# uthree/tinyvc

Measured on AMD Instinct MI355X. Metric: audio-samples/sec (16 kHz) end-to-end VC, higher is better.
Workload: dtype f32 (fp32 in / out / accumulate; channel contractions as two-term fp16 splits on v_mfma_f32_32x32x16_f16: 22-bit significands, three part-products per fp32 product)

## Files before the change

### tinyvc_amd/csrc/conv48s.hip

```cpp
#include "small_kernels.h"
#include "split_fp16.h"
#include "tvc_common.h"

namespace tvc {

namespace {

constexpr int kC48 = 48, kBN48 = 128, kXP48 = kBN48 + 2 * 27, kNT48 = 512;
typedef float f32x4s_t __attribute__((ext_vector_type(4)));
typedef unsigned u32x2_t __attribute__((ext_vector_type(2)));

__device__ __forceinline__ void split4_48(const float (&v)[4], u32x2_t& p1, u32x2_t& p2) {
#pragma unroll
    for (int j = 0; j < 2; ++j) {
        unsigned q1, q2;
        split2(v[2 * j], v[2 * j + 1], q1, q2);
        p1[j] = q1;
        p2[j] = q2;
    }
}

__device__ __forceinline__ void ld8_g8(float (&dst)[8], const float* base, unsigned byte_off) {
    const uint4* b4 = reinterpret_cast<const uint4*>(base);
    const f32x4s_t q0 = __builtin_bit_cast(f32x4s_t, ldg_so4(b4, byte_off)), q1 = __builtin_bit_cast(f32x4s_t, ldg_so4(b4, byte_off + 16u));
    dst[0] = q0.x; dst[1] = q0.y; dst[2] = q0.z; dst[3] = q0.w;
    dst[4] = q1.x; dst[5] = q1.y; dst[6] = q1.z; dst[7] = q1.w;
}
__device__ __forceinline__ void ld4_g8(float (&dst)[4], const float* base, unsigned byte_off) {
    const f32x4s_t q0 = __builtin_bit_cast(f32x4s_t, ldg_so4(reinterpret_cast<const uint4*>(base), byte_off));
    dst[0] = q0.x; dst[1] = q0.y; dst[2] = q0.z; dst[3] = q0.w;
}

struct Conv48Args {
    const float* x;
    const float* cond;
    const float* res;
    float* out;
    const u32x4* A6;
    const u32x4* F6;
    const u32x4* W5;
    const float* b5;
    float* out5;
    const float* bias;
    const float* bsc;
    const float* bsh;
    const float* wsc;
    const float* fsc;
    const float* w5sc;
    const float* amax_x;
    const float* amax_c;
    float* amax_y;
    int len, dil, tiles_per_utt, ntiles;
    RagDev rag;
};

template <bool FILM, bool C5 = false, bool RAG = false>
__global__ __launch_bounds__(kNT48) __attribute__((amdgpu_waves_per_eu(FILM ? 2 : 4))) void conv48s_kernel(Conv48Args a) {
    constexpr int C = kC48, BN = kBN48, XP = kXP48, NT = kNT48;
    extern __shared__ __attribute__((aligned(16))) uint4 smem_q[];
    u32x4* Xs = reinterpret_cast<u32x4*>(smem_q);
// ... 8 lines not shown
    const int XW = BN + 2 * dil;
    int bh = 0;
    auto utt = [&](int tile) __attribute__((always_inline)) { return rag_tile<RAG>(a.rag, tile, a.tiles_per_utt, rs, bh).b; };

    for (int i = tid; i < 36 * 64; i += NT) Wt[i] = a.A6[i];
    if (FILM)
        for (int i = tid; i < 24 * 64; i += NT) Ft[i] = a.F6[i];
    if (C5) {
        for (int i = tid; i < 6 * 64; i += NT) W5t[i] = a.W5[i];
        if (tid < 32) Bi[192 + tid] = a.b5[tid];
        if (tid == 0) Bi[224] = 0.f;
    }
    if (tid < 64) {
        const int tc = tid < C ? tid : C - 1;
        Bi[tid] = a.bias[tc];
        if (FILM) {
            Bi[64 + tid] = a.bsc[tc];
            Bi[128 + tid] = a.bsh[tc];
        }
    }
    const float cw = a.wsc[mt], cwsc = FILM ? a.fsc[mt] : 1.f, cwsh = FILM ? a.fsc[2 + mt] : 1.f, cw5 = C5 ? a.w5sc[0] : 1.f;

    constexpr int XPER = 3;
    float xr0[XPER][8];
    int ig[XPER], ic[XPER];
#pragma unroll
    for (int i = 0; i < XPER; ++i) {
        const int idx = tid + i * NT;
        const int g = idx / XW;
        ic[i] = idx - g * XW;
        ig[i] = g;
    }
    auto fetch = [&](int tile) __attribute__((always_inline)) {
        const RagTile rt = rag_tile<RAG>(a.rag, tile, a.tiles_per_utt, rs, bh);
        const int len = rt.len;
        const int px0 = rt.tin * BN - dil;
        const float* xb = RAG ? a.x + 8L * rt.off : a.x + (long)rt.b * C * rs;
#pragma unroll
        for (int i = 0; i < XPER; ++i) {
            const int g = ig[i] > 5 ? 5 : ig[i];
            int p = px0 + ic[i];
            p = p < 0 ? 0 : (p > len - 1 ? len - 1 : p);
            ld8_g8(xr0[i], xb, 32u * (unsigned)(g * rs + p));
        }
    };
    auto deposit = [&](float xs) __attribute__((always_inline)) {
#pragma unroll
        for (int i = 0; i < XPER; ++i) {
            if (ig[i] > 5) continue;
            float v[8];
#pragma unroll
            for (int j = 0; j < 8; ++j) {
                const float t = xr0[i][j];
                v[j] = fmaxf(t, 0.1f * t) * xs;
            }
            uint4 p1, p2;
            split8(v, p1, p2);
            Xs[(0 + ig[i]) * XP + ic[i]] = __builtin_bit_cast(u32x4, p1);
            Xs[(6 + ig[i]) * XP + ic[i]] = __builtin_bit_cast(u32x4, p2);
        }
    };

    int tile, tend;
    tile_range(a.ntiles, tile, tend);
    if (tile >= tend) return;
    bh = utt(tile);
    fetch(tile);
    deposit(bfp_load_u(a.amax_x, bh).s);
    slab_barrier();
    float mx_run = 0.f;
    int mx_b = bh;
    int sc_b = -1;
    Bfp sx{1.f, 1.f}, sc{1.f, 1.f};

    for (; tile < tend; ++tile) {
        const RagTile rt = rag_tile<RAG>(a.rag, tile, a.tiles_per_utt, rs, bh);
        const int b = rt.b, len = rt.len;
        bh = b;
        if (a.amax_y && b != mx_b) {
            amax_flush_wg(a.amax_y + mx_b, mx_run, Bi + 228);
            mx_run = 0.f;
            mx_b = b;
        }
        if (b != sc_b) {
            sc_b = b;
            sx = bfp_load_u(a.amax_x, b);
            sc = FILM ? bfp_load_u(a.amax_c, b) : Bfp{1.f, 1.f};
        }
        const int t0 = rt.tin * BN;
        const int next = tile + 1;
        const int n = nt * 32 + l31;
        const int t = t0 + n;
        const int tc = t < len ? t : len - 1;

        float cr[FILM ? 3 : 1][8];
        if (FILM) {
            const float* cb = RAG ? a.cond + 8L * rt.off : a.cond + (long)b * C * rs;
            const unsigned oc = 32u * (unsigned)(lh * rs + tc);
#pragma unroll
            for (int s = 0; s < 3; ++s) ld8_g8(cr[s], cb + (long)s * 16 * rs, oc);
        }
        float rv[FILM ? 4 : 1][4];
        if constexpr (FILM) {
            const float* rb = RAG ? a.res + 8L * rt.off : a.res + (long)b * C * rs;
            const unsigned og = 32u * (unsigned)(4 * mt * rs + tc) + 16u * (unsigned)lh;
#pragma unroll
            for (int g = 0; g < 4; ++g) {
                if (32 * mt + 8 * g < C) {
                    ld4_g8(rv[g], rb + (long)g * 8 * rs, og);
// ... 52 lines not shown
#pragma unroll
                for (int p = 0; p < 2; ++p) {
                    fa[0][p] = __builtin_bit_cast(f16x8, Ft[((s * 4 + mt) * 2 + p) * 64 + lane]);
                    fa[1][p] = __builtin_bit_cast(f16x8, Ft[((s * 4 + 2 + mt) * 2 + p) * 64 + lane]);
                }
                lsc = TVC_MFMA16(fa[0][1], cf[0], lsc);
                lsh = TVC_MFMA16(fa[1][1], cf[0], lsh);
                asc = TVC_MFMA16(fa[0][0], cf[0], asc);
                ash = TVC_MFMA16(fa[1][0], cf[0], ash);
                lsc = TVC_MFMA16(fa[0][0], cf[1], lsc);
                lsh = TVC_MFMA16(fa[1][0], cf[1], lsh);
            }
            const float c1 = cwsc * sc.inv, c2 = cwsh * sc.inv;
#pragma unroll
            for (int r = 0; r < 16; ++r) {
                asc[r] = comb(asc[r], lsc[r], c1, c1 * kLoInv);
                ash[r] = comb(ash[r], lsh[r], c2, c2 * kLoInv);
            }
        }

        float xv[C5 ? 4 : 1][4];
        float mx = 0.f;
        {
            float* ob = C5 ? nullptr : (RAG ? a.out + 8L * rt.off : a.out + (long)b * C * rs);
            const unsigned og = 32u * (unsigned)(4 * mt * rs + tc) + 16u * (unsigned)lh;
#pragma unroll
            for (int g = 0; g < 4; ++g) {
                if (32 * mt + 8 * g >= C) continue;
                float v4[4];
                const f32x4s_t bv = *reinterpret_cast<const f32x4s_t*>(Bi + 32 * mt + 8 * g + 4 * lh);
                f32x4s_t bs, bh;
                if (FILM) {
                    bs = *reinterpret_cast<const f32x4s_t*>(Bi + 64 + 32 * mt + 8 * g + 4 * lh);
                    bh = *reinterpret_cast<const f32x4s_t*>(Bi + 128 + 32 * mt + 8 * g + 4 * lh);
                }
#pragma unroll
                for (int q = 0; q < 4; ++q) {
                    float v = acc[4 * g + q] + bv[q];
                    if (FILM) {
                        v = __fadd_rn(__fmul_rn(v, asc[4 * g + q] + bs[q]), ash[4 * g + q] + bh[q]);
                        v = __fadd_rn(v, rv[g][q]);
                    }
                    v4[q] = v;
                    if (C5) {
                        xv[g][q] = v;
                        mx = fmaxf(mx, fabsf(v));
                    }
                }
                if (!C5 && t < len) {
                    stg_so4(ob + (long)g * 8 * rs, og, v4);
                    mx = fmaxf(mx, fmaxf(fmaxf(fabsf(v4[0]), fabsf(v4[1])), fmaxf(fabsf(v4[2]), fabsf(v4[3]))));
                }
            }
        }
        if (!C5) mx_run = fmaxf(mx_run, mx);
        if (C5) {
            {
#pragma unroll
                for (int o = 32; o > 0; o >>= 1) mx = fmaxf(mx, __shfl_xor(mx, o));
                if (lane == 0) atomicMax(reinterpret_cast<unsigned*>(Bi + 224), __builtin_bit_cast(unsigned, mx));
            }
            slab_barrier();
            const Bfp s5 = bfp_from_amax(Bi[224]);
#pragma unroll
            for (int g = 0; g < 4; ++g) {
                if (32 * mt + 8 * g >= C) continue;
                u32x2_t p1, p2;
#pragma unroll
                for (int q = 0; q < 4; ++q) xv[g][q] *= s5.s;
                split4_48(xv[g], p1, p2);
                const auto sx_ = __builtin_amdgcn_permlane32_swap(p1[0], p2[0], false, false);
                const auto sy_ = __builtin_amdgcn_permlane32_swap(p1[1], p2[1], false, false);
                const u32x4 row = {sx_[0], sy_[0], sx_[1], sy_[1]};
                *reinterpret_cast<u32x4*>(Xs + (6 * lh + 4 * mt + g) * XP + n) = row;
// ... 19 lines not shown
                float m5 = 0.f;
                if (t < len) {
                    float* o5 = RAG ? a.out5 + 8L * rt.off : a.out5 + (long)b * 24 * rs;
                    const unsigned o5o = 32u * (unsigned)t + 16u * (unsigned)lh;
                    const float c = cw5 * s5.inv, cl = c * kLoInv;
#pragma unroll
                    for (int g = 0; g < 3; ++g) {
                        const f32x4s_t b5v = *reinterpret_cast<const f32x4s_t*>(Bi + 192 + 8 * g + 4 * lh);
                        float v4[4];
#pragma unroll
                        for (int q = 0; q < 4; ++q) {
                            v4[q] = comb(a5[4 * g + q], l5[4 * g + q], c, cl) + b5v[q];
                            m5 = fmaxf(m5, fabsf(v4[q]));
                        }
                        stg_so4(o5 + (long)g * 8 * rs, o5o, v4);
                    }
                }
                mx_run = fmaxf(mx_run, m5);
            }
        }
        slab_barrier();
        if (next < tend) {
            const int bn = utt(next);
            deposit(bn == b ? sx.s : bfp_load_u(a.amax_x, bn).s);
        }
        slab_barrier();
    }
    if (a.amax_y) amax_flush_wg(a.amax_y + mx_b, mx_run, Bi + 228);
}

template <bool FILM, bool C5 = false>
int launch48(tvc_ctx* ctx, hipStream_t s, Conv48Args a, int B) {
    constexpr size_t lds = (size_t)(12 * kXP48 + 36 * 64 + (FILM ? 24 * 64 : 0) + (C5 ? 6 * 64 : 0)) * 16 + 240 * 4;
    TVC_CHECK((lds_optin<conv48s_kernel<FILM, C5>, conv48s_kernel<FILM, C5, true>>(ctx, (int)lds, "conv48s")));
    a.tiles_per_utt = (a.len + kBN48 - 1) / kBN48;
    a.ntiles = a.tiles_per_utt * B;
    TVC_CHECK(rag_tiles(ctx, s, B, a.len, kBN48, &a.rag, &a.ntiles, "conv48s"));
    const int wpc = FILM ? 1 : 2;
    const int grid = a.ntiles < wpc * ctx->ncu ? a.ntiles : wpc * ctx->ncu;
    if (ctx->rag) hipLaunchKernelGGL((conv48s_kernel<FILM, C5, true>), dim3(grid), dim3(kNT48), lds, s, a);
    else hipLaunchKernelGGL((conv48s_kernel<FILM, C5>), dim3(grid), dim3(kNT48), lds, s, a);
    return launch_check(ctx, "conv48s");
}

struct Conv48PArgs {
    const float* x;
    const float* cond;
    float* out;
    const u32x4* Aa;
    const u32x4* Ab;
    const u32x4* F6;
    const float *bias_a, *bias_b, *bsc, *bsh;
    const float *wsc_a, *wsc_b, *fsc;
    const float* amax_x;
    const float* amax_c;
    float* amax_y;
    RagDev rag;
    int len, da, db, lin, tiles_per_utt, ntiles;
    float lscale;
};
constexpr int kXPP = 136;

template <bool FILM, bool RAG = false>
__global__ __launch_bounds__(kNT48) __attribute__((amdgpu_waves_per_eu(2))) void conv48p_kernel(Conv48PArgs a) {
    constexpr int C = kC48, NT = kNT48, XP = kXPP, HP = 128;
    extern __shared__ __attribute__((aligned(16))) uint4 smem_p[];
    u32x4* Xs = reinterpret_cast<u32x4*>(smem_p);
    u32x4* Hs = Xs + 12 * XP;
    u32x4* Wa = Hs + 12 * HP;
    u32x4* Wb = Wa + 36 * 64;
    u32x4* Ft = Wb + 36 * 64;
    float* Bi = reinterpret_cast<float*>(Ft + (FILM ? 24 * 64 : 0));
    const int tid = threadIdx.x, lane = tid & 63, wave = tid >> 6;
    const int l31 = lane & 31, lh = lane >> 5;
    const int mt = wave >> 2, nt = wave & 3;
    const int rs = a.len, da = a.da, db = a.db;
    const int BNO = 128 - 2 * db;
    const int XW = 128 + 2 * da;
    const int rsl = FILM ? a.lin : rs;
    const int xf = FILM ? rs / a.lin : 1;
    int bh = 0;
    auto utt = [&](int tile) __attribute__((always_inline)) { return rag_tile<RAG>(a.rag, tile, a.tiles_per_utt, rs, bh).b; };

    for (int i = tid; i < 36 * 64; i += NT) {
        Wa[i] = a.Aa[i];
        Wb[i] = a.Ab[i];
    }
    if (FILM)
        for (int i = tid; i < 24 * 64; i += NT) Ft[i] = a.F6[i];
    if (tid < 64) {
        const int tc = tid < C ? tid : C - 1;
        Bi[tid] = a.bias_a[tc];
        Bi[64 + tid] = a.bias_b[tc];
        if (FILM) {
            Bi[128 + tid] = a.bsc[tc];
            Bi[192 + tid] = a.bsh[tc];
        }
    }
    if (tid == 0) Bi[256] = 0.f;
    const int mtu = __builtin_amdgcn_readfirstlane(mt);
    const float cwa = a.wsc_a[mtu], cwb = a.wsc_b[mtu], cwsc = FILM ? a.fsc[mtu] : 1.f, cwsh = FILM ? a.fsc[2 + mtu] : 1.f;

    constexpr int XPER = 2;
    float xr0[XPER][8], xr1[FILM ? XPER : 1][8], lam[FILM ? XPER : 1];
    int ig[XPER], ic[XPER];
#pragma unroll
    for (int i = 0; i < XPER; ++i) {
        const int idx = tid + i * NT;
        const int g = idx / XW;
        ic[i] = idx - g * XW;
        ig[i] = g;
    }
    auto fetch = [&](int tile) __attribute__((always_inline)) {
        const RagTile rt = rag_tile<RAG>(a.rag, tile, a.tiles_per_utt, rs, bh);
        const int len = rt.len, lin = FILM ? len / xf : len;
        const int px0 = rt.tin * BNO - db - da;
        const float* xb = RAG ? a.x + (FILM ? 8L * (rt.off / xf) : rt.off) : a.x + (long)rt.b * C * rsl;
#pragma unroll
        for (int i = 0; i < XPER; ++i) {
            const int g = ig[i] > 5 ? 5 : ig[i];
            int p = px0 + ic[i];
            p = p < 0 ? 0 : (p > len - 1 ? len - 1 : p);
// ... 20 lines not shown
            float v[8];
#pragma unroll
            for (int j = 0; j < 8; ++j) {
                float t = FILM ? fmaf(1.f - lam[i], xr0[i][j], __fmul_rn(lam[i], xr1[i][j])) : xr0[i][j];
                v[j] = fmaxf(t, 0.1f * t) * xs;
            }
            uint4 p1, p2;
            split8(v, p1, p2);
            Xs[(0 + g) * XP + c] = __builtin_bit_cast(u32x4, p1);
            Xs[(6 + g) * XP + c] = __builtin_bit_cast(u32x4, p2);
        }
    };

    int tile, tend;
    tile_range(a.ntiles, tile, tend);
    if (tile >= tend) return;
    bh = utt(tile);
    fetch(tile);
    deposit(bfp_load_u(a.amax_x, bh).s);
    slab_barrier();
    float mx_run = 0.f;
    int mx_b = bh;
    int sc_b = -1;
    Bfp sx{1.f, 1.f}, sc{1.f, 1.f};

    for (; tile < tend; ++tile) {
        const RagTile rt = rag_tile<RAG>(a.rag, tile, a.tiles_per_utt, rs, bh);
        const int b = rt.b, len = rt.len;
        bh = b;
        if (a.amax_y && b != mx_b) {
            amax_flush_wg(a.amax_y + mx_b, mx_run, Bi + 260);
            mx_run = 0.f;
            mx_b = b;
        }
        if (b != sc_b) {
            sc_b = b;
            sx = bfp_load_u(a.amax_x, b);
            sc = FILM ? bfp_load_u(a.amax_c, b) : Bfp{1.f, 1.f};
        }
        const int t0 = rt.tin * BNO;
        const int next = tile + 1;
        const int n = nt * 32 + l31;
        const int t = t0 + n;
        const bool live = n < BNO && t < len;
        const int tc = t < len ? t : len - 1;
        const unsigned oo = 4u * (unsigned)((32 * mt + 4 * lh) * rs + tc);

        float cr[FILM ? 3 : 1][8];
        if (FILM) {
            const float* cb = RAG ? a.cond + 8L * rt.off : a.cond + (long)b * C * rs;
            const unsigned oc = 32u * (unsigned)(lh * rs + tc);
#pragma unroll
            for (int s = 0; s < 3; ++s) ld8_g8(cr[s], cb + (long)s * 16 * rs, oc);
        }
        float rv[FILM ? 4 : 1][4];
        if constexpr (FILM) {
            const float* rb = RAG ? a.x + 8L * (rt.off / xf) : a.x + (long)b * C * a.lin;
            const Lerp lc = lerp_coord(tc, a.lscale, RAG ? len / xf : a.lin);
            const unsigned o0 = 32u * (unsigned)(4 * mt * a.lin + lc.i0) + 16u * (unsigned)lh, o1 = 32u * (unsigned)(4 * mt * a.lin + lc.i1) + 16u * (unsigned)lh;
#pragma unroll
// ... 15 lines not shown
            f16x8 af[2][2], bf[2][2];
            auto frags = [&](int s, int fb) __attribute__((always_inline)) {
                const int sl = s / 3, tap = s - sl * 3;
                const int row = (2 * sl + lh) * XP + n + tap * da;
#pragma unroll
                for (int p = 0; p < 2; ++p) {
                    bf[fb][p] = __builtin_bit_cast(f16x8, Xs[p * 6 * XP + row]);
                    af[fb][p] = __builtin_bit_cast(f16x8, Wa[((s * 2 + mt) * 2 + p) * 64 + lane]);
                }
            };
            frags(0, 0);
#pragma unroll
            for (int s = 0; s < 9; ++s) {
                const int fb = s & 1;
                if (s + 1 < 9) frags(s + 1, fb ^ 1);
                __builtin_amdgcn_sched_barrier(0);
                alo = TVC_MFMA16(af[fb][1], bf[fb][0], alo);
                acc = TVC_MFMA16(af[fb][0], bf[fb][0], acc);
                alo = TVC_MFMA16(af[fb][0], bf[fb][1], alo);
                __builtin_amdgcn_sched_barrier(0);
            }
        }
        fetch(next < tend ? next : tile);
        float hv[4][4];
        float hmx = 0.f;
        {
            const float c = cwa * sx.inv, cl = c * kLoInv;
#pragma unroll
            for (int g = 0; g < 4; ++g) {
                const f32x4s_t bv = *reinterpret_cast<const f32x4s_t*>(Bi + 32 * mt + 8 * g + 4 * lh);
#pragma unroll
                for (int q = 0; q < 4; ++q) {
                    const float v = comb(acc[4 * g + q], alo[4 * g + q], c, cl) + bv[q];
                    hv[g][q] = fmaxf(v, 0.1f * v);
                    if (32 * mt + 8 * g < C) hmx = fmaxf(hmx, fabsf(hv[g][q]));
                }
            }
            hmx = wave_max(hmx);
            if (lane == 0) atomicMax(reinterpret_cast<unsigned*>(Bi + 256), __builtin_bit_cast(unsigned, hmx));
        }
        slab_barrier();
        const Bfp sh_ = bfp_from_amax(Bi[256]);
#pragma unroll
        for (int g = 0; g < 4; ++g) {
            if (32 * mt + 8 * g >= C) continue;
            u32x2_t p1, p2;
#pragma unroll
            for (int q = 0; q < 4; ++q) hv[g][q] *= sh_.s;
            split4_48(hv[g], p1, p2);
            const auto sx_ = __builtin_amdgcn_permlane32_swap(p1[0], p2[0], false, false);
            const auto sy_ = __builtin_amdgcn_permlane32_swap(p1[1], p2[1], false, false);
            const u32x4 row = {sx_[0], sy_[0], sx_[1], sy_[1]};
            *reinterpret_cast<u32x4*>(Hs + (6 * lh + 4 * mt + g) * HP + n) = row;
        }
        slab_barrier();
        if (tid == 0) Bi[256] = 0.f;

#pragma unroll
        for (int r = 0; r < 16; ++r) acc[r] = alo[r] = 0.f;
        {
            const int lo = db - t0 > 0 ? db - t0 : 0;
            const int hi = len - 1 - t0 + db < HP - 1 ? len - 1 - t0 + db : HP - 1;
            int col[3];
#pragma unroll
            for (int tap = 0; tap < 3; ++tap) {
                int c = n + tap * db;
                c = c > HP - 1 ? HP - 1 : c;
                col[tap] = c < lo ? lo : (c > hi ? hi : c);
            }
            f16x8 af[2][2], bf[2][2];
            auto frags = [&](int s, int fb) __attribute__((always_inline)) {
                const int sl = s / 3, tap = s - sl * 3;
                const int row = (2 * sl + lh) * HP + col[tap];
#pragma unroll
                for (int p = 0; p < 2; ++p) {
                    bf[fb][p] = __builtin_bit_cast(f16x8, Hs[p * 6 * HP + row]);
                    af[fb][p] = __builtin_bit_cast(f16x8, Wb[((s * 2 + mt) * 2 + p) * 64 + lane]);
                }
            };
// ... 64 lines not shown
                for (int q = 0; q < 4; ++q) {
                    float v = acc[4 * g + q] + bv[q];
                    if (FILM) {
                        v = __fadd_rn(__fmul_rn(v, asc[4 * g + q] + bs[q]), ash[4 * g + q] + bh[q]);
                        v = __fadd_rn(v, rv[g][q]);
                    }
                    v4[q] = v;
                    if (!FILM && live) stg_so(ob + (long)(8 * g + q) * rs, oo, v);
                }
                if (live) {
                    if (FILM) stg_so4(ob + (long)g * 8 * rs, og, v4);
                    mx = fmaxf(mx, fmaxf(fmaxf(fabsf(v4[0]), fabsf(v4[1])), fmaxf(fabsf(v4[2]), fabsf(v4[3]))));
                }
            }
            mx_run = fmaxf(mx_run, mx);
        }
        slab_barrier();
        if (next < tend) {
            const int bn = utt(next);
            deposit(bn == b ? sx.s : bfp_load_u(a.amax_x, bn).s);
        }
        slab_barrier();
    }
    if (a.amax_y) amax_flush_wg(a.amax_y + mx_b, mx_run, Bi + 260);
}

template <bool FILM>
int launch48p(tvc_ctx* ctx, hipStream_t s, Conv48PArgs a, int B) {
    constexpr size_t lds = (size_t)(12 * kXPP + 12 * 128 + 72 * 64 + (FILM ? 24 * 64 : 0)) * 16 + 272 * 4;
    static_assert(lds <= 160 * 1024, "LDS");
    TVC_CHECK((lds_optin<conv48p_kernel<FILM>, conv48p_kernel<FILM, true>>(ctx, (int)lds, "conv48p")));
    const int bno = 128 - 2 * a.db;
    a.tiles_per_utt = (a.len + bno - 1) / bno;
    a.ntiles = a.tiles_per_utt * B;
    TVC_CHECK(rag_tiles(ctx, s, B, a.len, bno, &a.rag, &a.ntiles, "conv48p"));
    const int grid = a.ntiles < ctx->ncu ? a.ntiles : ctx->ncu;
    if (ctx->rag) hipLaunchKernelGGL((conv48p_kernel<FILM, true>), dim3(grid), dim3(kNT48), lds, s, a);
    else hipLaunchKernelGGL((conv48p_kernel<FILM>), dim3(grid), dim3(kNT48), lds, s, a);
    return launch_check(ctx, "conv48p");
}

}

int run_conv48s(tvc_ctx* ctx, hipStream_t s, const PackedW& w, const float* x, const PackedW* film, const float* bsc, const float* bsh,
                const float* cond, const float* res, float* out, int B, int len, int dil, const float* amax_x, const float* amax_c, float* amax_y,
                const PackedW* c5, float* out5) {
    if (w.cin != kC48 || w.M != kC48 || w.taps != 3 || w.MT6 != 2 || !w.A6) return fail(ctx, TVC_ERR_ARG, "conv48s: 48 -> 48 channel k3 convs only");
    if (dil < 1 || dil > 27) return fail(ctx, TVC_ERR_ARG, "conv48s: dilation must be 1..27");
    if ((long)len * kC48 * 4 >= (1L << 32)) return fail(ctx, TVC_ERR_ARG, "conv48s: utterance too long for 32-bit byte offsets");
    if (film && (film->MT6 != 4 || !film->A6 || !cond || !bsc || !bsh)) return fail(ctx, TVC_ERR_ARG, "conv48s: FiLM needs the stacked image, both biases and cond");
    Conv48Args a{};
    a.x = x; a.cond = cond; a.res = res; a.out = out;
    a.A6 = reinterpret_cast<const u32x4*>(w.A6);
    a.F6 = film ? reinterpret_cast<const u32x4*>(film->A6) : nullptr;
    a.bias = w.bias; a.bsc = bsc; a.bsh = bsh;
    a.wsc = w.wscale;
    a.fsc = film ? film->wscale : nullptr;
    a.amax_x = amax_x; a.amax_c = amax_c; a.amax_y = amax_y;
    a.len = len; a.dil = dil;
    if (film) {
        if (!res) return fail(ctx, TVC_ERR_ARG, "conv48s: the FiLM variants carry a residual");
        if (c5) {
            if (!out5 || c5->M != 24 || c5->cin != kC48 || c5->taps != 1 || c5->MT6 != 1 || !c5->A6)
                return fail(ctx, TVC_ERR_ARG, "conv48s: the fused c5 is the 48 -> 24 1x1 after the second FiLM");
            a.W5 = reinterpret_cast<const u32x4*>(c5->A6);
            a.b5 = c5->bias;
            a.w5sc = c5->wscale;
            a.out5 = out5;
            return launch48<true, true>(ctx, s, a, B);
        }
        return launch48<true>(ctx, s, a, B);
    }
    if (res) return fail(ctx, TVC_ERR_ARG, "conv48s: plain convs carry no residual");
    return launch48<false>(ctx, s, a, B);
}

int run_conv48_pair(tvc_ctx* ctx, hipStream_t s, const PackedW& wa, const PackedW& wb, const float* x, int lin, float lscale, const PackedW* film,
                    const float* bsc, const float* bsh, const float* cond, float* out, int B, int len, int da, int db, const float* amax_x,
                    const float* amax_c, float* amax_y) {
    for (const PackedW* w : {&wa, &wb})
        if (w->cin != kC48 || w->M != kC48 || w->taps != 3 || w->MT6 != 2 || !w->A6) return fail(ctx, TVC_ERR_ARG, "conv48 pair: 48 -> 48 channel k3 convs only");
    if (da < 1 || da > 4 || db < 1 || db > 8) return fail(ctx, TVC_ERR_ARG, "conv48 pair: dilations (1..4, 1..8)");
    if ((long)len * kC48 * 4 >= (1L << 32)) return fail(ctx, TVC_ERR_ARG, "conv48 pair: utterance too long for 32-bit byte offsets");
    if (film && (film->MT6 != 4 || !film->A6 || !cond || !bsc || !bsh))
        return fail(ctx, TVC_ERR_ARG, "conv48 pair: the FiLM variant needs the stacked image, both biases and cond");
    Conv48PArgs a{};
    a.x = x; a.cond = cond; a.out = out;
    a.Aa = reinterpret_cast<const u32x4*>(wa.A6);
    a.Ab = reinterpret_cast<const u32x4*>(wb.A6);
    a.F6 = film ? reinterpret_cast<const u32x4*>(film->A6) : nullptr;
    a.bias_a = wa.bias; a.bias_b = wb.bias; a.bsc = bsc; a.bsh = bsh;
    a.wsc_a = wa.wscale; a.wsc_b = wb.wscale; a.fsc = film ? film->wscale : nullptr;
    a.amax_x = amax_x; a.amax_c = amax_c; a.amax_y = amax_y;
    a.len = len; a.da = da; a.db = db; a.lin = lin; a.lscale = lscale;
    if (film) return lin > 0 ? launch48p<true>(ctx, s, a, B) : fail(ctx, TVC_ERR_ARG, "conv48 pair: the FiLM pair starts from the low-rate tensor");
    if (lin > 0) return fail(ctx, TVC_ERR_ARG, "conv48 pair: the plain pair has no interpolated input");
    return launch48p<false>(ctx, s, a, B);
}

}
```

### tinyvc_amd/csrc/decoder.hip

```cpp
#include "conv3s.h"
#include "conv_s2.h"
#include "film_s2.h"
#include "gemm_s2.h"
#include "small_kernels.h"
#include "tvc_common.h"

namespace tvc {


__device__ __forceinline__ float div24k(float x) {
    const float r = 1.0f / 24000.0f;
    const float q0 = __fmul_rn(x, r);
    return fmaf(fmaf(-q0, 24000.0f, x), r, q0);
}

__device__ __forceinline__ double wave_incl_scan(double v, int lane) {
#pragma unroll
    for (int o = 1; o < 64; o <<= 1) {
        double u = __shfl_up(v, o);
        if (lane >= o) v += u;
    }
    return v;
}

// ... 329 lines not shown
            }
            TVC_CHECK(fk->end());
        }
        TVC_CHECK(run_down0_split(ctx, s, ctx->flt_down0s, source, energy, skip[0], taps ? taps->skips[0] : nullptr, xi_pre[1], B, (int)L, smax, slot(S_SKIP0)));
    }
    for (int i = 1; i <= 4; ++i) {
        const DownW& d = ctx->downs[i - 1];
        const int len = (int)len_dn[i];
        size_t mk = ws.mark();
        float* xi = xi_pre[i];
        float* h1 = d.cin == 24 ? nullptr : ws.get<float>((size_t)B * d.cin * len);
        float* h2 = d.cin == 24 ? nullptr : ws.get<float>((size_t)B * d.cin * len);
        if (!ws.dry) {
            static const char* names[4] = {"filter.down1", "filter.down2", "filter.down3", "filter.down4"};
            ProfScope ps(ctx, s, ws, names[i - 1]);
            float* y2 = i < 4 ? xi_pre[i + 1] : nullptr;
            const int f2 = i < 4 ? ctx->downs[i].factor : 0;
            const float* mxi = slot(S_SKIP0 + i - 1);
            float *mh1 = slot(S_DH1 + i - 1), *mh2 = slot(S_DH2 + i - 1), *mout = slot(S_SKIP0 + i);
            if (d.cin == 24) {
                TVC_CHECK(run_down24_fused(ctx, s, d, xi, skip[i], y2, B, len, mxi, mout));
            } else {
                if (d.cin == 48) {
                    TVC_CHECK(run_conv48_pair(ctx, s, d.c1, d.c2, xi, 0, 0.f, nullptr, nullptr, nullptr, nullptr, h2, B, len, 1, 2, mxi, nullptr, mh2));
                } else {
                    TVC_CHECK(plain_conv(ctx, s, d.c1, xi, B, d.cin, len, 1, h1, BfpSlots{mxi, nullptr, mh1}));
                    TVC_CHECK(plain_conv(ctx, s, d.c2, h1, B, d.cin, len, 2, h2, BfpSlots{mh1, nullptr, mh2}));
                }
                TVC_CHECK((conv3s_launch<true, C3EpiBiasResConv>(ctx, s, d.c3, h2, B, d.cin, len, 4,
                                                                 C3EpiBiasResConv{{skip[i], d.c3res_bias, nullptr, d.cout, len, y2, f2}},
                                                                 BfpSlots{mh2, mxi, mout}, &d.res, nullptr, xi, d.cin)));
            }
        }
        ws.release(mk);
    }
    float* xlev[5];
    {
        long l = T;
        for (int i = 0; i < 5; ++i) {
            l *= ctx->ups[i].factor;
            xlev[i] = ws.get<float>((size_t)B * ctx->ups[i].cout * l);
        }
    }
    long len = T;
    const float* mx_in = slot(S_X);
    for (int i = 0; i < 5; ++i) {
        const UpW& u = ctx->ups[i];
// ... 6 lines not shown
        float* xu = ws.get<float>((size_t)B * C * lo);
        float* h = i == 0 ? h0 : ws.get<float>((size_t)B * C * lo);
        float* x1 = ws.get<float>((size_t)B * C * lo);
        if (!ws.dry && C == 24) {
            ProfScope ps(ctx, s, ws, "filter.up4+out");
            TVC_CHECK(run_up24_split(ctx, s, u, x, cond, ctx->down0_bw, ctx->down0_bb, x1, wave, B, lo, mx_in, smax, slot(S_UX1 + i)));
        } else if (!ws.dry) {
            static const char* names[4] = {"filter.up0", "filter.up1", "filter.up2", "filter.up3"};
            ProfScope ps(ctx, s, ws, names[i]);
            const float lscale = (float)(1.0 / (double)u.factor);
            for (int half = 0; half < 2; ++half) {
                const PackedW& ca = half ? u.c3 : u.c1;
                const PackedW& cb = half ? u.c4 : u.c2;
                const PackedW& fw = half ? u.film2 : u.film1;
                const float* bsc = fw.bias;
                const float* bsh = fw.bias + C;
                const int da = kHalfDil[half][0], db = kHalfDil[half][1];
                float* xout = half ? xu : x1;
                const float* ma_in = half ? slot(S_UX1 + i) : mx_in;
                float* mh = slot((half ? S_UHB : S_UHA) + i);
                float* mout = slot((half ? S_UXU : S_UX1) + i);
                if (C == 48) {
                    if (half == 0) {
                        TVC_CHECK(run_conv48_pair(ctx, s, ca, cb, x, lin, lscale, &fw, bsc, bsh, cond, xout, B, lo, da, db, ma_in, mcond, mout));
                    } else {
                        TVC_CHECK(run_conv48s(ctx, s, ca, x1, nullptr, nullptr, nullptr, nullptr, nullptr, h, B, lo, da, ma_in, nullptr, mh));
                        TVC_CHECK(run_conv48s(ctx, s, cb, h, &fw, bsc, bsh, cond, x1, nullptr, B, lo, db, mh, mcond, slot(S_LEV + i), &u.c5, xlev[i]));
                    }
                } else if (half == 0 && i == 0) {
                    if (fk) TVC_CHECK(fk->join());
                    else TVC_CHECK(up0_first(s));
                    TVC_CHECK(half_film(ctx, s, cb, fw, u.fu1, db, h, cond, B, C, lo, xout, bsc, bsh, x, lin, lscale, ma_in, mh, mcond, mout, pre0));
                } else if (half == 0) {
                    TVC_CHECK(conv_film_half(ctx, s, ca, cb, fw, u.fu1, x, lin, lscale, da, db, h, cond, B, C, lo, xout, bsc, bsh, x, lin, lscale, ma_in, mh, mcond, mout));
                } else {
                    TVC_CHECK(conv_film_half(ctx, s, ca, cb, fw, u.fu2, x1, 0, 0.f, da, db, h, cond, B, C, lo, xout, bsc, bsh, x1, 0, 0.f, ma_in, mh, mcond, mout));
                }
            }
            if (C != 48) {
                EpiBias<ACT_NONE, false> ep{xlev[i], u.c5.bias, nullptr, u.cout, lo, nc, (long)u.cout * lo, 0, slot(S_LEV + i), slot(S_UXU + i), u.c5_bw, u.c5_bb, NB};
                if (u.cout == 48) {
                    EpiBiasG8 eg{xlev[i], u.c5.bias, u.cout, lo, nc, slot(S_LEV + i), slot(S_UXU + i), u.c5_bw, u.c5_bb, NB};
                    TVC_CHECK((gemm_s_launch<2, 4, 2>(ctx, s, u.c5, xu, B, C, lo, 0, eg, slot(S_UXU + i))));
                } else if (u.c5.MT6 % 3 == 0) TVC_CHECK((gemm_s_launch<3, 4, 1>(ctx, s, u.c5, xu, B, C, lo, 0, ep, slot(S_UXU + i))));
                else TVC_CHECK((gemm_s_launch<2, 4, 2>(ctx, s, u.c5, xu, B, C, lo, 0, ep, slot(S_UXU + i))));
            }
        }
        ws.release(mk);
        x = xlev[i];
        mx_in = slot(S_LEV + i);
// ... 78 lines not shown
```

### tinyvc_amd/csrc/pack.hip

```cpp
#include <algorithm>
#include <cmath>

#include "tvc_common.h"

namespace tvc {

size_t ArenaBuilder::put(const float** slot, const float* v, size_t n) {
    const size_t off = (buf.size() + 63) & ~size_t(63);
    buf.resize(off + n, 0.f);
    std::copy(v, v + n, buf.begin() + off);
    fix.push_back({slot, off});
    return off;
}

namespace {

int pad_m(int M) {
    if (M <= 32) return 32;
    if (M <= 64) return 64;
    if (M <= 96) return 96;
    if (M % 96 == 0 && M % 128 != 0) return M;
    return (M + 127) / 128 * 128;
}

// ... 427 lines not shown
        if (fw && fb) {
            const RowL1 r = row_l1(fw, fb, ch[0], 1);
            ctx->flt_in_bb += (float)((r.w * 89.0 + r.b) * 1.0001);
        }
    }
    pk.down0s(&ctx->flt_down0s, "filter_net.downs.0", &ctx->down0_bw, &ctx->down0_bb);
    for (int i = 1; i <= 4; ++i) {
        DownW& d = ctx->downs[i - 1];
        d.cin = ch[5 - i];
        d.cout = ch[4 - i];
        d.factor = fac[5 - i];
        std::string p = "filter_net.downs." + std::to_string(i);
        pk.conv_joint(p + ".c3", &d.c3, d.cin, 3, p + ".down_res", &d.res, d.cin, 1);
        if (d.cin == 24) {
            pk.conv24s(&d.s24c1, p + ".c1", 24);
            pk.conv24s(&d.s24c2, p + ".c2", 24);
            pk.conv24s(&d.s24c3r, p + ".c3", 48, p + ".down_res.bias", &d.c3);
            pk.bound(p + ".c1", 24, 72, &d.b1_w, &d.b1_b);
            pk.bound(p + ".c2", 24, 72, &d.b2_w, &d.b2_b);
            continue;
        }
        pk.conv({p + ".c1"}, &d.c1, d.cin, 3);
        pk.conv({p + ".c2"}, &d.c2, d.cin, 3);
        const float* b3 = pk.get(p + ".c3.bias", d.cout);
        const float* br = pk.get(p + ".down_res.bias", d.cout);
        if (b3 && br) {
            std::vector<float> sum(d.c3.Mpad, 0.f);
            for (int m = 0; m < d.cout; ++m) sum[m] = b3[m] + br[m];
            ab->put(&d.c3res_bias, sum);
        }
    }
    for (int i = 0; i < 5; ++i) {
        UpW& u = ctx->ups[i];
        u.cin = ch[i];
        u.cout = i < 4 ? ch[i + 1] : ch[4];
        u.factor = fac[i];
        std::string p = "filter_net.ups." + std::to_string(i);
        if (u.cin == 24) {
            pk.up24s_half(&u.s24a, p + ".c1", p + ".c2", p + ".film1", "", "");
            pk.up24s_half(&u.s24b, p + ".c3", p + ".c4", p + ".film2", p + ".c5", "filter_net.output_layer");
            continue;
        }
        pk.conv({p + ".c1"}, &u.c1, u.cin, 3);
        pk.conv({p + ".c2"}, &u.c2, u.cin, 3);
        pk.conv({p + ".c3"}, &u.c3, u.cin, 3);
        pk.conv({p + ".c4"}, &u.c4, u.cin, 3);
        pk.conv({p + ".c5"}, &u.c5, u.cin, 1);
        pk.bound(p + ".c5", u.cout, u.cin, &u.c5_bw, &u.c5_bb);
        pk.conv({p + ".film1.to_scale", p + ".film1.to_shift"}, &u.film1, u.cin, 1);
        pk.conv({p + ".film2.to_scale", p + ".film2.to_shift"}, &u.film2, u.cin, 1);
        if (u.cin >= 96) {
            pk.film_u(&u.fu1, p + ".c2", p + ".film1", u.cin, p + ".c1");
            pk.film_u(&u.fu2, p + ".c4", p + ".film2", u.cin, p + ".c3");
        }
    }
    *missing_dec = pk.missing;
}

}
```

### tinyvc_amd/csrc/tvc_common.h

```cpp
#pragma once
#include <hip/hip_runtime.h>

#include <atomic>
#include <cstdarg>
#include <cstdint>
#include <cstdio>
#include <cstring>
#include <map>
#include <string>
#include <vector>

#include "../../include/tinyvc_hip.h"
#include "ragged.h"

namespace tvc {

constexpr int kSampleRate = 24000;
constexpr int kNfft = 1920;
constexpr int kHop = 480;
constexpr int kBins = 961;
constexpr int kSslDim = 768;
constexpr int kSslCh = 384;
constexpr int kPitchCh = 128;
constexpr int kPitchClasses = 512;
// ... 47 lines not shown
};

struct DownW {
    PackedW res, c1, c2, c3;
    const float* c3res_bias = nullptr;
    const float* s24c1 = nullptr;
    const float* s24c2 = nullptr;
    const float* s24c3r = nullptr;
    float b1_w = 0.f, b1_b = 0.f, b2_w = 0.f, b2_b = 0.f;
    int cin = 0, cout = 0, factor = 1;
};
struct FilmU {
    static constexpr int TAB_BIAS = 0, TAB_SCALE = 1, TAB_BSC = 2, TAB_BSH = 3, TAB_SSC = 4, TAB_SSH = 5;
    const float* img = nullptr;
    const float* tab = nullptr;
    int C = 0;
    float hb_w = 0.f, hb_b = 0.f;
};
struct UpW {
    PackedW c1, c2, c3, c4, c5, film1, film2;
    FilmU fu1, fu2;
    const float* s24a = nullptr;
    const float* s24b = nullptr;
    float c5_bw = 0.f, c5_bb = 0.f;
    int cin = 0, cout = 0, factor = 1;
};

struct HostTensor {
    std::vector<float> data;
    std::vector<int64_t> shape;
};

struct ArenaBuilder {
    std::vector<float> buf;
    std::vector<std::pair<const float**, size_t>> fix;
    size_t put(const float** slot, const float* v, size_t n);
    size_t put(const float** slot, const std::vector<float>& v) { return put(slot, v.data(), v.size()); }
    void resolve(const float* arena) const {
        for (auto& f : fix) *f.first = arena + f.second;
    }
};

}

struct tvc_prof_region {
    std::string name;
// ... 382 lines not shown
int run_stream_resample(tvc_ctx*, hipStream_t, const void* in, bool in16, void* out, bool out16, float* state, int S, int64_t n_in, int in_freq,
                        int out_freq, float gain_db);
int run_pcm16_to_f32(tvc_ctx*, hipStream_t, const int16_t* pcm, float* y, int64_t n, float gain_db);
int run_f32_to_pcm16(tvc_ctx*, hipStream_t, const float* x, int16_t* pcm, int64_t n, float gain_db);
void frontdoor_release(tvc_ctx*);
int run_prepare_index(tvc_ctx*, hipStream_t, const float* index, float* prepared, int64_t N);
int run_prepare_index_f16(tvc_ctx*, hipStream_t, const void* rows_f16, float* prepared, int64_t N);
int run_prepare_index_cols(tvc_ctx*, hipStream_t, const float* feats, int64_t S, const int64_t* cols, int64_t N, float* prepared, float* index_out);
int run_prepare_index_cols_f16(tvc_ctx*, hipStream_t, const float* feats, int64_t S, const int64_t* cols, int64_t N, float* prepared, void* index_out_f16);

constexpr int kIndexAssignChunk = 32768;
constexpr int64_t kIndexCompactMaxK = 1 << 20;
int run_index_assign(tvc_ctx*, hipStream_t, Ws&, const float* points, int64_t N, const float* cent_blob, int64_t K, int64_t* assign, float* sim_out, int32_t* moved);
int run_index_update(tvc_ctx*, hipStream_t, Ws&, const float* points, int64_t N, const int64_t* assign, int64_t K, float* centroids, int32_t* counts_out);
int run_index_compact(tvc_ctx*, hipStream_t, Ws&, const float* points, int64_t N, const int64_t* init_cols, int64_t K, int iters, float* centroids, float* prepared_out,
                      int64_t* assign_out, int32_t* counts_out, int32_t* moved_out);

int run_up24_split(tvc_ctx*, hipStream_t, const UpW& u, const float* x, const float* cond_planes, float cbw, float cbb, float* x1, float* out, int B, int len,
                   const float* amax_x, const float* amax_c, float* amax_x1);
int run_down0_split(tvc_ctx*, hipStream_t, const float* blob, const float* source, const float* energy, float* planes, float* out_fp32, float* y2, int B, int len,
                    const float* amax_x, float* amax_y);
int run_down24_fused(tvc_ctx*, hipStream_t, const DownW& d, const float* xi, float* out, float* y2, int B, int len, const float* amax_xi, float* amax_out);
int run_conv48s(tvc_ctx*, hipStream_t, const PackedW& w, const float* x, const PackedW* film, const float* bsc, const float* bsh, const float* cond,
                const float* res, float* out, int B, int len, int dil, const float* amax_x, const float* amax_c, float* amax_y,
                const PackedW* c5 = nullptr, float* out5 = nullptr);

int run_conv48_pair(tvc_ctx*, hipStream_t, const PackedW& wa, const PackedW& wb, const float* x, int lin, float lscale, const PackedW* film, const float* bsc,
                    const float* bsh, const float* cond, float* out, int B, int len, int da, int db, const float* amax_x, const float* amax_c,
                    float* amax_y);

int run_convnext(tvc_ctx*, hipStream_t, Ws&, const ConvNeXtW& w, float* x, int B, int T, float* amax_out = nullptr);

}
```

Baseline: 712.6 million.

## Use weight-derived static bounds for intermediate scales instead of measured maxima

```diff
diff --git a/tinyvc_amd/csrc/conv48s.hip b/tinyvc_amd/csrc/conv48s.hip
--- a/tinyvc_amd/csrc/conv48s.hip
+++ b/tinyvc_amd/csrc/conv48s.hip
@@ -26,6 +26,12 @@
     dst[0] = q0.x; dst[1] = q0.y; dst[2] = q0.z; dst[3] = q0.w;
     dst[4] = q1.x; dst[5] = q1.y; dst[6] = q1.z; dst[7] = q1.w;
 }
+__device__ __forceinline__ void stg_so4u(uint4* base, unsigned byte_off, u32x4 v) {
+    typedef __attribute__((address_space(1))) u32x4* gu4;
+    gu4 p = (gu4)base;
+    asm("" : "+s"(p));
+    *reinterpret_cast<gu4>(reinterpret_cast<__attribute__((address_space(1))) char*>(p) + byte_off) = v;
+}
 __device__ __forceinline__ void ld4_g8(float (&dst)[4], const float* base, unsigned byte_off) {
     const f32x4s_t q0 = __builtin_bit_cast(f32x4s_t, ldg_so4(reinterpret_cast<const uint4*>(base), byte_off));
     dst[0] = q0.x; dst[1] = q0.y; dst[2] = q0.z; dst[3] = q0.w;
@@ -33,9 +39,12 @@
 
 struct Conv48Args {
     const float* x;
+    const uint4* xpre;
     const float* cond;
     const float* res;
     float* out;
+    uint4* opre;
+    float pre_w, pre_b;
     const u32x4* A6;
     const u32x4* F6;
     const u32x4* W5;
@@ -90,7 +99,8 @@
     const float cw = a.wsc[mt], cwsc = FILM ? a.fsc[mt] : 1.f, cwsh = FILM ? a.fsc[2 + mt] : 1.f, cw5 = C5 ? a.w5sc[0] : 1.f;
 
     constexpr int XPER = 3;
-    float xr0[XPER][8];
+    float xr0[FILM ? 1 : XPER][8];
+    u32x4 xq[FILM ? XPER : 1][2];
     int ig[XPER], ic[XPER];
 #pragma unroll
     for (int i = 0; i < XPER; ++i) {
@@ -104,28 +114,40 @@
         const int len = rt.len;
         const int px0 = rt.tin * BN - dil;
         const float* xb = RAG ? a.x + 8L * rt.off : a.x + (long)rt.b * C * rs;
+        const uint4* xp = RAG ? a.xpre + rt.off : a.xpre + (long)rt.b * 12 * rs;
 #pragma unroll
         for (int i = 0; i < XPER; ++i) {
             const int g = ig[i] > 5 ? 5 : ig[i];
             int p = px0 + ic[i];
             p = p < 0 ? 0 : (p > len - 1 ? len - 1 : p);
-            ld8_g8(xr0[i], xb, 32u * (unsigned)(g * rs + p));
+            if constexpr (FILM) {
+                const unsigned o = 16u * (unsigned)(g * rs + p);
+                xq[i][0] = ldg_so4(xp, o);
+                xq[i][1] = ldg_so4(xp + 6L * rs, o);
+            } else {
+                ld8_g8(xr0[i], xb, 32u * (unsigned)(g * rs + p));
+            }
         }
     };
     auto deposit = [&](float xs) __attribute__((always_inline)) {
 #pragma unroll
         for (int i = 0; i < XPER; ++i) {
             if (ig[i] > 5) continue;
-            float v[8];
-#pragma unroll
-            for (int j = 0; j < 8; ++j) {
-                const float t = xr0[i][j];
-                v[j] = fmaxf(t, 0.1f * t) * xs;
-            }
-            uint4 p1, p2;
-            split8(v, p1, p2);
-            Xs[(0 + ig[i]) * XP + ic[i]] = __builtin_bit_cast(u32x4, p1);
-            Xs[(6 + ig[i]) * XP + ic[i]] = __builtin_bit_cast(u32x4, p2);
+            if constexpr (FILM) {
+                Xs[(0 + ig[i]) * XP + ic[i]] = xq[i][0];
+                Xs[(6 + ig[i]) * XP + ic[i]] = xq[i][1];
+            } else {
+                float v[8];
+#pragma unroll
+                for (int j = 0; j < 8; ++j) {
+                    const float t = xr0[i][j];
+                    v[j] = fmaxf(t, 0.1f * t) * xs;
+                }
+                uint4 p1, p2;
+                split8(v, p1, p2);
+                Xs[(0 + ig[i]) * XP + ic[i]] = __builtin_bit_cast(u32x4, p1);
+                Xs[(6 + ig[i]) * XP + ic[i]] = __builtin_bit_cast(u32x4, p2);
+            }
         }
     };
 
@@ -134,12 +156,12 @@
     if (tile >= tend) return;
     bh = utt(tile);
     fetch(tile);
-    deposit(bfp_load_u(a.amax_x, bh).s);
+    deposit(FILM ? 1.f : bfp_load_u(a.amax_x, bh).s);
     slab_barrier();
     float mx_run = 0.f;
     int mx_b = bh;
     int sc_b = -1;
-    Bfp sx{1.f, 1.f}, sc{1.f, 1.f};
+    Bfp sx{1.f, 1.f}, sc{1.f, 1.f}, sp{1.f, 1.f};
 
     for (; tile < tend; ++tile) {
         const RagTile rt = rag_tile<RAG>(a.rag, tile, a.tiles_per_utt, rs, bh);
@@ -152,7 +174,9 @@
         }
         if (b != sc_b) {
             sc_b = b;
-            sx = bfp_load_u(a.amax_x, b);
+            const float slot_x = sload_f32(a.amax_x + b);
+            sp = bfp_from_amax(fmaf(a.pre_w, slot_x, a.pre_b));
+            sx = FILM ? sp : bfp_from_amax(slot_x);
             sc = FILM ? bfp_load_u(a.amax_c, b) : Bfp{1.f, 1.f};
         }
         const int t0 = rt.tin * BN;
@@ -251,8 +275,10 @@
         float xv[C5 ? 4 : 1][4];
         float mx = 0.f;
         {
-            float* ob = C5 ? nullptr : (RAG ? a.out + 8L * rt.off : a.out + (long)b * C * rs);
+            float* ob = C5 || !FILM ? nullptr : (RAG ? a.out + 8L * rt.off : a.out + (long)b * C * rs);
             const unsigned og = 32u * (unsigned)(4 * mt * rs + tc) + 16u * (unsigned)lh;
+            uint4* pb = FILM ? nullptr : (RAG ? a.opre + rt.off : a.opre + (long)b * 12 * rs);
+            const unsigned op = 16u * (unsigned)((6 * lh + 4 * mt) * rs + tc);
 #pragma unroll
             for (int g = 0; g < 4; ++g) {
                 if (32 * mt + 8 * g >= C) continue;
@@ -276,9 +302,17 @@
                         mx = fmaxf(mx, fabsf(v));
                     }
                 }
-                if (!C5 && t < len) {
-                    stg_so4(ob + (long)g * 8 * rs, og, v4);
-                    mx = fmaxf(mx, fmaxf(fmaxf(fabsf(v4[0]), fabsf(v4[1])), fmaxf(fabsf(v4[2]), fabsf(v4[3]))));
+                if (FILM && !C5 && t < len) stg_so4(ob + (long)g * 8 * rs, og, v4);
+                if (!C5 && t < len) mx = fmaxf(mx, fmaxf(fmaxf(fabsf(v4[0]), fabsf(v4[1])), fmaxf(fabsf(v4[2]), fabsf(v4[3]))));
+                if constexpr (!FILM) {
+                    float hv[4];
+#pragma unroll
+                    for (int q = 0; q < 4; ++q) hv[q] = fmaxf(v4[q], 0.1f * v4[q]) * sp.s;
+                    u32x2_t p1, p2;
+                    split4_48(hv, p1, p2);
+                    const auto qx = __builtin_amdgcn_permlane32_swap(p1[0], p2[0], false, false);
+                    const auto qy = __builtin_amdgcn_permlane32_swap(p1[1], p2[1], false, false);
+                    if (t < len) stg_so4u(pb + (long)g * rs, op, u32x4{qx[0], qy[0], qx[1], qy[1]});
                 }
             }
         }
@@ -344,7 +378,7 @@
         slab_barrier();
         if (next < tend) {
             const int bn = utt(next);
-            deposit(bn == b ? sx.s : bfp_load_u(a.amax_x, bn).s);
+            deposit(FILM || bn == b ? sx.s : bfp_load_u(a.amax_x, bn).s);
         }
         slab_barrier();
     }
@@ -380,6 +414,7 @@
     RagDev rag;
     int len, da, db, lin, tiles_per_utt, ntiles;
     float lscale;
+    float ha_w, ha_b;
 };
 constexpr int kXPP = 136;
 
@@ -419,7 +454,6 @@
             Bi[192 + tid] = a.bsh[tc];
         }
     }
-    if (tid == 0) Bi[256] = 0.f;
     const int mtu = __builtin_amdgcn_readfirstlane(mt);
     const float cwa = a.wsc_a[mtu], cwb = a.wsc_b[mtu], cwsc = FILM ? a.fsc[mtu] : 1.f, cwsh = FILM ? a.fsc[2 + mtu] : 1.f;
 
@@ -486,20 +520,22 @@
     float mx_run = 0.f;
     int mx_b = bh;
     int sc_b = -1;
-    Bfp sx{1.f, 1.f}, sc{1.f, 1.f};
+    Bfp sx{1.f, 1.f}, sc{1.f, 1.f}, sh_{1.f, 1.f};
 
     for (; tile < tend; ++tile) {
         const RagTile rt = rag_tile<RAG>(a.rag, tile, a.tiles_per_utt, rs, bh);
         const int b = rt.b, len = rt.len;
         bh = b;
         if (a.amax_y && b != mx_b) {
-            amax_flush_wg(a.amax_y + mx_b, mx_run, Bi + 260);
+            amax_flush_wg(a.amax_y + mx_b, mx_run, Bi + 256);
             mx_run = 0.f;
             mx_b = b;
         }
         if (b != sc_b) {
             sc_b = b;
-            sx = bfp_load_u(a.amax_x, b);
+            const float slot_x = sload_f32(a.amax_x + b);
+            sx = bfp_from_amax(slot_x);
+            sh_ = bfp_from_amax(fmaf(a.ha_w, slot_x, a.ha_b));
             sc = FILM ? bfp_load_u(a.amax_c, b) : Bfp{1.f, 1.f};
         }
         const int t0 = rt.tin * BNO;
@@ -561,39 +597,27 @@
             }
         }
         fetch(next < tend ? next : tile);
-        float hv[4][4];
-        float hmx = 0.f;
         {
             const float c = cwa * sx.inv, cl = c * kLoInv;
 #pragma unroll
             for (int g = 0; g < 4; ++g) {
+                if (32 * mt + 8 * g >= C) continue;
                 const f32x4s_t bv = *reinterpret_cast<const f32x4s_t*>(Bi + 32 * mt + 8 * g + 4 * lh);
+                float hv[4];
 #pragma unroll
                 for (int q = 0; q < 4; ++q) {
                     const float v = comb(acc[4 * g + q], alo[4 * g + q], c, cl) + bv[q];
-                    hv[g][q] = fmaxf(v, 0.1f * v);
-                    if (32 * mt + 8 * g < C) hmx = fmaxf(hmx, fabsf(hv[g][q]));
-                }
-            }
-            hmx = wave_max(hmx);
-            if (lane == 0) atomicMax(reinterpret_cast<unsigned*>(Bi + 256), __builtin_bit_cast(unsigned, hmx));
+                    hv[q] = fmaxf(v, 0.1f * v) * sh_.s;
+                }
+                u32x2_t p1, p2;
+                split4_48(hv, p1, p2);
+                const auto sx_ = __builtin_amdgcn_permlane32_swap(p1[0], p2[0], false, false);
+                const auto sy_ = __builtin_amdgcn_permlane32_swap(p1[1], p2[1], false, false);
+                const u32x4 row = {sx_[0], sy_[0], sx_[1], sy_[1]};
+                *reinterpret_cast<u32x4*>(Hs + (6 * lh + 4 * mt + g) * HP + n) = row;
+            }
         }
         slab_barrier();
-        const Bfp sh_ = bfp_from_amax(Bi[256]);
-#pragma unroll
-        for (int g = 0; g < 4; ++g) {
-            if (32 * mt + 8 * g >= C) continue;
-            u32x2_t p1, p2;
-#pragma unroll
-            for (int q = 0; q < 4; ++q) hv[g][q] *= sh_.s;
-            split4_48(hv[g], p1, p2);
-            const auto sx_ = __builtin_amdgcn_permlane32_swap(p1[0], p2[0], false, false);
-            const auto sy_ = __builtin_amdgcn_permlane32_swap(p1[1], p2[1], false, false);
-            const u32x4 row = {sx_[0], sy_[0], sx_[1], sy_[1]};
-            *reinterpret_cast<u32x4*>(Hs + (6 * lh + 4 * mt + g) * HP + n) = row;
-        }
-        slab_barrier();
-        if (tid == 0) Bi[256] = 0.f;
 
 #pragma unroll
         for (int r = 0; r < 16; ++r) acc[r] = alo[r] = 0.f;
@@ -704,12 +728,12 @@
         }
         slab_barrier();
     }
-    if (a.amax_y) amax_flush_wg(a.amax_y + mx_b, mx_run, Bi + 260);
+    if (a.amax_y) amax_flush_wg(a.amax_y + mx_b, mx_run, Bi + 256);
 }
 
 template <bool FILM>
 int launch48p(tvc_ctx* ctx, hipStream_t s, Conv48PArgs a, int B) {
-    constexpr size_t lds = (size_t)(12 * kXPP + 12 * 128 + 72 * 64 + (FILM ? 24 * 64 : 0)) * 16 + 272 * 4;
+    constexpr size_t lds = (size_t)(12 * kXPP + 12 * 128 + 72 * 64 + (FILM ? 24 * 64 : 0)) * 16 + 264 * 4;
     static_assert(lds <= 160 * 1024, "LDS");
     TVC_CHECK((lds_optin<conv48p_kernel<FILM>, conv48p_kernel<FILM, true>>(ctx, (int)lds, "conv48p")));
     const int bno = 128 - 2 * a.db;
@@ -726,13 +750,22 @@
 
 int run_conv48s(tvc_ctx* ctx, hipStream_t s, const PackedW& w, const float* x, const PackedW* film, const float* bsc, const float* bsh,
                 const float* cond, const float* res, float* out, int B, int len, int dil, const float* amax_x, const float* amax_c, float* amax_y,
-                const PackedW* c5, float* out5) {
+                float pre_w, float pre_b, const PackedW* c5, float* out5) {
     if (w.cin != kC48 || w.M != kC48 || w.taps != 3 || w.MT6 != 2 || !w.A6) return fail(ctx, TVC_ERR_ARG, "conv48s: 48 -> 48 channel k3 convs only");
     if (dil < 1 || dil > 27) return fail(ctx, TVC_ERR_ARG, "conv48s: dilation must be 1..27");
     if ((long)len * kC48 * 4 >= (1L << 32)) return fail(ctx, TVC_ERR_ARG, "conv48s: utterance too long for 32-bit byte offsets");
     if (film && (film->MT6 != 4 || !film->A6 || !cond || !bsc || !bsh)) return fail(ctx, TVC_ERR_ARG, "conv48s: FiLM needs the stacked image, both biases and cond");
+    if (!amax_x || !(pre_w > 0.f)) return fail(ctx, TVC_ERR_STATE, "conv48s: the bound of the plain conv's output (and its input's |max| slot) is missing");
     Conv48Args a{};
-    a.x = x; a.cond = cond; a.res = res; a.out = out;
+    a.cond = cond; a.res = res;
+    if (film) {
+        a.xpre = reinterpret_cast<const uint4*>(x);
+        a.out = out;
+    } else {
+        a.x = x;
+        a.opre = reinterpret_cast<uint4*>(out);
+    }
+    a.pre_w = pre_w; a.pre_b = pre_b;
     a.A6 = reinterpret_cast<const u32x4*>(w.A6);
     a.F6 = film ? reinterpret_cast<const u32x4*>(film->A6) : nullptr;
     a.bias = w.bias; a.bsc = bsc; a.bsh = bsh;
@@ -759,13 +792,14 @@
 
 int run_conv48_pair(tvc_ctx* ctx, hipStream_t s, const PackedW& wa, const PackedW& wb, const float* x, int lin, float lscale, const PackedW* film,
                     const float* bsc, const float* bsh, const float* cond, float* out, int B, int len, int da, int db, const float* amax_x,
-                    const float* amax_c, float* amax_y) {
+                    const float* amax_c, float* amax_y, float ha_w, float ha_b) {
     for (const PackedW* w : {&wa, &wb})
         if (w->cin != kC48 || w->M != kC48 || w->taps != 3 || w->MT6 != 2 || !w->A6) return fail(ctx, TVC_ERR_ARG, "conv48 pair: 48 -> 48 channel k3 convs only");
     if (da < 1 || da > 4 || db < 1 || db > 8) return fail(ctx, TVC_ERR_ARG, "conv48 pair: dilations (1..4, 1..8)");
     if ((long)len * kC48 * 4 >= (1L << 32)) return fail(ctx, TVC_ERR_ARG, "conv48 pair: utterance too long for 32-bit byte offsets");
     if (film && (film->MT6 != 4 || !film->A6 || !cond || !bsc || !bsh))
         return fail(ctx, TVC_ERR_ARG, "conv48 pair: the FiLM variant needs the stacked image, both biases and cond");
+    if (!amax_x || !(ha_w > 0.f)) return fail(ctx, TVC_ERR_STATE, "conv48 pair: the bound of the first conv's output (and its input's |max| slot) is missing");
     Conv48PArgs a{};
     a.x = x; a.cond = cond; a.out = out;
     a.Aa = reinterpret_cast<const u32x4*>(wa.A6);
@@ -775,6 +809,7 @@
     a.wsc_a = wa.wscale; a.wsc_b = wb.wscale; a.fsc = film ? film->wscale : nullptr;
     a.amax_x = amax_x; a.amax_c = amax_c; a.amax_y = amax_y;
     a.len = len; a.da = da; a.db = db; a.lin = lin; a.lscale = lscale;
+    a.ha_w = ha_w; a.ha_b = ha_b;
     if (film) return lin > 0 ? launch48p<true>(ctx, s, a, B) : fail(ctx, TVC_ERR_ARG, "conv48 pair: the FiLM pair starts from the low-rate tensor");
     if (lin > 0) return fail(ctx, TVC_ERR_ARG, "conv48 pair: the plain pair has no interpolated input");
     return launch48p<false>(ctx, s, a, B);
diff --git a/tinyvc_amd/csrc/decoder.hip b/tinyvc_amd/csrc/decoder.hip
--- a/tinyvc_amd/csrc/decoder.hip
+++ b/tinyvc_amd/csrc/decoder.hip
@@ -375,7 +375,7 @@
                 TVC_CHECK(run_down24_fused(ctx, s, d, xi, skip[i], y2, B, len, mxi, mout));
             } else {
                 if (d.cin == 48) {
-                    TVC_CHECK(run_conv48_pair(ctx, s, d.c1, d.c2, xi, 0, 0.f, nullptr, nullptr, nullptr, nullptr, h2, B, len, 1, 2, mxi, nullptr, mh2));
+                    TVC_CHECK(run_conv48_pair(ctx, s, d.c1, d.c2, xi, 0, 0.f, nullptr, nullptr, nullptr, nullptr, h2, B, len, 1, 2, mxi, nullptr, mh2, d.b1_w, d.b1_b));
                 } else {
                     TVC_CHECK(plain_conv(ctx, s, d.c1, xi, B, d.cin, len, 1, h1, BfpSlots{mxi, nullptr, mh1}));
                     TVC_CHECK(plain_conv(ctx, s, d.c2, h1, B, d.cin, len, 2, h2, BfpSlots{mh1, nullptr, mh2}));
@@ -428,10 +428,10 @@
                 float* mout = slot((half ? S_UXU : S_UX1) + i);
                 if (C == 48) {
                     if (half == 0) {
-                        TVC_CHECK(run_conv48_pair(ctx, s, ca, cb, x, lin, lscale, &fw, bsc, bsh, cond, xout, B, lo, da, db, ma_in, mcond, mout));
+                        TVC_CHECK(run_conv48_pair(ctx, s, ca, cb, x, lin, lscale, &fw, bsc, bsh, cond, xout, B, lo, da, db, ma_in, mcond, mout, u.c1_bw, u.c1_bb));
                     } else {
-                        TVC_CHECK(run_conv48s(ctx, s, ca, x1, nullptr, nullptr, nullptr, nullptr, nullptr, h, B, lo, da, ma_in, nullptr, mh));
-                        TVC_CHECK(run_conv48s(ctx, s, cb, h, &fw, bsc, bsh, cond, x1, nullptr, B, lo, db, mh, mcond, slot(S_LEV + i), &u.c5, xlev[i]));
+                        TVC_CHECK(run_conv48s(ctx, s, ca, x1, nullptr, nullptr, nullptr, nullptr, nullptr, h, B, lo, da, ma_in, nullptr, mh, u.c3_bw, u.c3_bb));
+                        TVC_CHECK(run_conv48s(ctx, s, cb, h, &fw, bsc, bsh, cond, x1, nullptr, B, lo, db, ma_in, mcond, slot(S_LEV + i), u.c3_bw, u.c3_bb, &u.c5, xlev[i]));
                     }
                 } else if (half == 0 && i == 0) {
                     if (fk) TVC_CHECK(fk->join());
diff --git a/tinyvc_amd/csrc/pack.hip b/tinyvc_amd/csrc/pack.hip
--- a/tinyvc_amd/csrc/pack.hip
+++ b/tinyvc_amd/csrc/pack.hip
@@ -473,6 +473,7 @@
         }
         pk.conv({p + ".c1"}, &d.c1, d.cin, 3);
         pk.conv({p + ".c2"}, &d.c2, d.cin, 3);
+        if (d.cin == 48) pk.bound(p + ".c1", 48, 144, &d.b1_w, &d.b1_b);
         const float* b3 = pk.get(p + ".c3.bias", d.cout);
         const float* br = pk.get(p + ".down_res.bias", d.cout);
         if (b3 && br) {
@@ -498,6 +499,10 @@
         pk.conv({p + ".c4"}, &u.c4, u.cin, 3);
         pk.conv({p + ".c5"}, &u.c5, u.cin, 1);
         pk.bound(p + ".c5", u.cout, u.cin, &u.c5_bw, &u.c5_bb);
+        if (u.cin == 48) {
+            pk.bound(p + ".c1", 48, 144, &u.c1_bw, &u.c1_bb);
+            pk.bound(p + ".c3", 48, 144, &u.c3_bw, &u.c3_bb);
+        }
         pk.conv({p + ".film1.to_scale", p + ".film1.to_shift"}, &u.film1, u.cin, 1);
         pk.conv({p + ".film2.to_scale", p + ".film2.to_shift"}, &u.film2, u.cin, 1);
         if (u.cin >= 96) {
diff --git a/tinyvc_amd/csrc/tvc_common.h b/tinyvc_amd/csrc/tvc_common.h
--- a/tinyvc_amd/csrc/tvc_common.h
+++ b/tinyvc_amd/csrc/tvc_common.h
@@ -93,6 +93,7 @@
     FilmU fu1, fu2;
     const float* s24a = nullptr;
     const float* s24b = nullptr;
+    float c1_bw = 0.f, c1_bb = 0.f, c3_bw = 0.f, c3_bb = 0.f;
     float c5_bw = 0.f, c5_bb = 0.f;
     int cin = 0, cout = 0, factor = 1;
 };
@@ -521,12 +522,12 @@
                     const float* amax_x, float* amax_y);
 int run_down24_fused(tvc_ctx*, hipStream_t, const DownW& d, const float* xi, float* out, float* y2, int B, int len, const float* amax_xi, float* amax_out);
 int run_conv48s(tvc_ctx*, hipStream_t, const PackedW& w, const float* x, const PackedW* film, const float* bsc, const float* bsh, const float* cond,
-                const float* res, float* out, int B, int len, int dil, const float* amax_x, const float* amax_c, float* amax_y,
+                const float* res, float* out, int B, int len, int dil, const float* amax_x, const float* amax_c, float* amax_y, float pre_w, float pre_b,
                 const PackedW* c5 = nullptr, float* out5 = nullptr);
 
 int run_conv48_pair(tvc_ctx*, hipStream_t, const PackedW& wa, const PackedW& wb, const float* x, int lin, float lscale, const PackedW* film, const float* bsc,
                     const float* bsh, const float* cond, float* out, int B, int len, int da, int db, const float* amax_x, const float* amax_c,
-                    float* amax_y);
+                    float* amax_y, float ha_w, float ha_b);
 
 int run_convnext(tvc_ctx*, hipStream_t, Ws&, const ConvNeXtW& w, float* x, int B, int T, float* amax_out = nullptr);
 
```

Result: no change. 716.0 million, median of 6 (+0.5%).
